# LuoGuiwen/MSM_blst

Measured on AMD Instinct MI355X. Metric: G1 MSM point-scalar pairs/sec at n=2^20, 1/2/4/8 MI355X; bit-exact vs CPU, higher is better.
Workload: dtype u32 (exact Fp381 integer arithmetic, 14x28-bit limbs)

## Files before the change

include/msm_mi355x.h:

```cpp
#ifndef MSM_MI355X_H
#define MSM_MI355X_H

#include <stddef.h>
#include <stdint.h>

#ifdef __cplusplus
extern "C" {
#endif

typedef uint8_t byte;
typedef uint64_t limb_t;
typedef struct { byte b[256 / 8]; } blst_scalar;
typedef struct { limb_t l[384 / 8 / sizeof(limb_t)]; } blst_fp;
typedef struct { blst_fp fp[2]; } blst_fp2;
typedef struct { blst_fp x, y, z; } blst_p1;
typedef struct { blst_fp x, y; } blst_p1_affine;
typedef struct { blst_fp2 x, y, z; } blst_p2;
typedef struct { blst_fp2 x, y; } blst_p2_affine;
typedef struct { blst_fp x, y, zzz, zz; } blst_p1xyzz;
typedef struct { blst_fp2 x, y, zzz, zz; } blst_p2xyzz;
typedef struct { int m; int b; int alpha; } digit_decomposition;

size_t blst_p1s_mult_pippenger_scratch_sizeof(size_t npoints);
void blst_p1s_mult_pippenger(blst_p1 *ret, const blst_p1_affine *const points[], size_t npoints,
// ... 242 lines not shown
                    const uint8_t *sig_codes, const uint8_t *key_codes, const uint8_t *late, const uint8_t *is_one,
                    uint8_t *status);

typedef struct { limb_t l[256 / 8 / sizeof(limb_t)]; } blst_fr;
enum { MSM_NTT_INVERSE = 1, MSM_FR_SRC_SCALAR = 2, MSM_FR_DST_SCALAR = 4 };
int msm_fr_ntt(int device, void *dst, const void *src, size_t log_n, size_t batch, const byte *shift, int flags,
               int src_on_device, int dst_on_device, void *hip_stream);
enum { MSM_FR_ADD, MSM_FR_SUB, MSM_FR_MUL, MSM_FR_SQR, MSM_FR_NEG, MSM_FR_INV, MSM_FR_FROM_SCALAR, MSM_FR_TO_SCALAR };
enum { MSM_FR_B_ONE = 1 };
int msm_fr_op(int device, int op, void *dst, const void *a, const void *b, size_t n, int flags, int src_on_device,
              int dst_on_device, void *hip_stream);
int msm_fr_root_of_unity(size_t log_n, blst_fr *out);
int msm_ntt_plan(size_t log_n, int *npasses, int log_radix[], int capacity);
int msm_fr_probe(int device, double out[2]);

enum { MSM_POLY_BITREV = 8 };
int msm_fr_eval_quotient(int device, void *y, void *q, const void *polys, const void *z, size_t log_n, size_t count,
                         int flags, int src_on_device, int dst_on_device, void *hip_stream);
typedef struct msm_kzg_ctx msm_kzg_ctx;
int msm_kzg_ctx_create(msm_kzg_ctx **ctx, int device, size_t log_n, const void *srs_lagrange_g1, int srs_on_device,
                       const void *tau_g2, int flags, void *hip_stream);
void msm_kzg_ctx_destroy(msm_kzg_ctx *ctx);
int msm_kzg_commit(msm_kzg_ctx *ctx, void *dst_affine, const void *polys, size_t count, int src_on_device,
                   int dst_on_device, void *hip_stream);
int msm_kzg_open(msm_kzg_ctx *ctx, void *proofs_affine, void *y, const void *polys, const void *z, size_t count,
                 int src_on_device, int dst_on_device, void *hip_stream);
int msm_kzg_verify(msm_kzg_ctx *ctx, uint8_t *ok, size_t *nfail, const void *commitments, const void *z,
                   const void *y, const void *proofs, size_t count, const byte *weights, size_t nbits,
                   size_t weight_stride, const size_t *batch_offsets, size_t nbatches, int src_on_device,
                   void *hip_stream);

size_t msm_ches_bucket_set(int q, int a_h, int *out, size_t cap);
int msm_ches_digit_table(int q, int a_h, digit_decomposition *out);

void msm_gen_scalars(byte *out32, size_t n, uint64_t seed);
void msm_p1_fixed_points(blst_p1_affine *out, size_t n);
void msm_p2_fixed_points(blst_p2_affine *out, size_t n);
void msm_p1_fixed_points_range(blst_p1_affine *out, size_t start, size_t n);
void msm_p2_fixed_points_range(blst_p2_affine *out, size_t start, size_t n);
void msm_p1_to_affine(blst_p1_affine *out, const blst_p1 *in);
void msm_p2_to_affine(blst_p2_affine *out, const blst_p2 *in);
void msm_p1_compress(byte out[48], const blst_p1 *in);
void msm_p2_compress(byte out[96], const blst_p2 *in);
void msm_p1_add(blst_p1 *out, const blst_p1 *a, const blst_p1 *b);
void msm_p2_add(blst_p2 *out, const blst_p2 *a, const blst_p2 *b);

int msm_test_field(int group, int op, const limb_t *a, const limb_t *b, limb_t *out, size_t n);
int msm_test_xyzz(int group, const void *points_affine, size_t npoints, const uint32_t *ops, int len, size_t nseq,
                  void *out);
int msm_test_fp12(int op, int k, int alias, int raw, const void *a, const void *b, void *out, size_t n);
int msm_test_fp_ops(int field, int form, int op, const uint32_t *in, const uint32_t *flags, uint32_t *out, size_t n,
                    size_t cap);

#ifdef __cplusplus
}
#endif
#endif
```

msm_blst_amd/_ffi.py:

```python
import ctypes
import os

HERE = os.path.dirname(os.path.abspath(__file__))
LIB_PATH = os.path.join(HERE, "libmsm_mi355x.so")

_lib = None


class MsmError(RuntimeError):
    pass


def lib():
    global _lib
    if _lib is not None:
        return _lib
    if not os.path.exists(LIB_PATH):
        raise MsmError(f"{LIB_PATH} not built: run `python -m msm_blst_amd.build` (hipcc, gfx950)")
    L = ctypes.CDLL(LIB_PATH)
    vp, sz, i32, u64 = ctypes.c_void_p, ctypes.c_size_t, ctypes.c_int, ctypes.c_uint64
    for g in (1, 2):
        f = getattr(L, f"blst_p{g}s_mult_pippenger")
        f.argtypes = [vp, vp, sz, vp, sz, vp]
        f.restype = None
        f = getattr(L, f"blst_p{g}s_tile_pippenger")
        f.argtypes = [vp, vp, sz, vp, sz, vp, sz, sz]
        f.restype = None
        f = getattr(L, f"blst_p{g}s_mult_pippenger_scratch_sizeof")
        f.argtypes = [sz]
        f.restype = sz
        getattr(L, f"msm_p{g}_fixed_points").argtypes = [vp, sz]
        getattr(L, f"msm_p{g}_fixed_points_range").argtypes = [vp, sz, sz]
        for name in (f"msm_p{g}_to_affine", f"msm_p{g}_compress"):
            getattr(L, name).argtypes = [vp, vp]
        getattr(L, f"msm_p{g}_add").argtypes = [vp, vp, vp]
    L.msm_last_error.restype = ctypes.c_char_p
    L.msm_device_count.restype = i32
    L.msm_ctx_create.argtypes = [ctypes.POINTER(vp), i32, i32, i32]
    L.msm_ctx_set_points.argtypes = [vp, vp, sz, i32, vp]
    L.msm_ctx_mult.argtypes = [vp, vp, vp, sz, sz, i32, vp]
    L.msm_ctx_mult_batch.argtypes = [vp, vp, vp, sz, sz, sz, sz, i32, vp]
    L.msm_ctx_set_profiling.argtypes = [vp, i32]
    L.msm_ctx_phase_times.argtypes = [vp, vp]
    L.msm_ctx_destroy.argtypes = [vp]
    L.msm_ctx_destroy.restype = None
    L.msm_gen_scalars.argtypes = [vp, sz, u64]
    L.msm_test_field.argtypes = [i32, i32, vp, vp, vp, sz]
    L.msm_test_xyzz.argtypes = [i32, vp, sz, vp, i32, sz, vp]
    L.msm_test_fp12.argtypes = [i32, i32, i32, i32, vp, vp, vp, sz]
    L.msm_test_fp_ops.argtypes = [i32, i32, i32, vp, vp, vp, sz, sz]
    pp = ctypes.POINTER(vp)
    L.msm_ches_params.argtypes = [i32, i32, vp]
    L.msm_ches_ctx_create.argtypes = [pp, i32, i32, i32, i32]
    L.msm_ches_ctx_create_params.argtypes = [pp, i32, i32, vp]
    L.msm_ches_ctx_create_multi.argtypes = [pp, i32, vp, i32, i32, i32]
    L.msm_ches_ctx_shards.argtypes = [vp]
    L.msm_ches_ctx_build_table.argtypes = [vp, vp, sz, i32, vp]
    L.msm_ches_ctx_set_table.argtypes = [vp, vp, sz, i32, vp]
    L.msm_ches_ctx_get_table.argtypes = [vp, vp, sz, sz]
    L.msm_ches_ctx_mult.argtypes = [vp, vp, vp, sz, i32, vp]
    L.msm_ches_ctx_mult_batch.argtypes = [vp, vp, vp, sz, sz, sz, i32, vp]
    L.msm_ches_ctx_set_profiling.argtypes = [vp, i32]
    L.msm_ches_ctx_phase_times.argtypes = [vp, vp]
    L.msm_ches_ctx_bucket_count.argtypes = [vp]
    L.msm_ches_ctx_bucket_count.restype = sz
    L.msm_register_host_table.argtypes = [i32, vp, sz]
    L.msm_unregister_host_table.argtypes = [vp]
    L.msm_ches_ctx_batch_lanes.argtypes = [vp]
    L.msm_ches_ctx_rccl_exchange.argtypes = [vp]
    L.msm_ches_ctx_time_accumulation.argtypes = [vp, vp, sz, i32, i32, vp]
    L.msm_ches_ctx_destroy.argtypes = [vp]
    L.msm_ches_ctx_destroy.restype = None
    L.msm_ches_bucket_set.argtypes = [i32, i32, vp, sz]
    L.msm_ches_bucket_set.restype = sz
    L.msm_ches_digit_table.argtypes = [i32, i32, vp]
    for g in (1, 2):
        f = getattr(L, f"blst_p{g}s_mult_wbits_precompute_sizeof")
        f.argtypes, f.restype = [sz, sz], sz
        f = getattr(L, f"blst_p{g}s_mult_wbits_scratch_sizeof")
        f.argtypes, f.restype = [sz], sz
        f = getattr(L, f"blst_p{g}s_mult_wbits_precompute")
        f.argtypes, f.restype = [vp, sz, vp, sz], None
        f = getattr(L, f"blst_p{g}s_mult_wbits")
        f.argtypes, f.restype = [vp, vp, sz, sz, vp, sz, vp], None
    if hasattr(L, "msm_release_engine_cache"):
        L.msm_release_engine_cache.argtypes = []
        L.msm_release_engine_cache.restype = None
        L.msm_engine_cache_stats.argtypes = [vp]
        L.msm_engine_cache_stats.restype = None
        L.msm_set_engine_cache_limit.argtypes = [sz]
        L.msm_set_engine_cache_limit.restype = sz
    L.msm_set_abort_on_error.argtypes = [i32]
    L.msm_error_pending.argtypes = []
    L.msm_wbits_ctx_create.argtypes = [pp, i32, i32, i32]
    L.msm_wbits_ctx_precompute.argtypes = [vp, vp, sz, i32, vp]
    L.msm_wbits_ctx_set_table.argtypes = [vp, vp, sz, i32, vp]
    L.msm_wbits_ctx_get_table.argtypes = [vp, vp, sz, sz]
    L.msm_wbits_ctx_mult.argtypes = [vp, vp, vp, sz, sz, i32, vp]
    L.msm_wbits_ctx_table_rows.argtypes = [vp]
    L.msm_wbits_ctx_table_rows.restype = sz
    L.msm_wbits_ctx_destroy.argtypes = [vp]
    L.msm_wbits_ctx_destroy.restype = None
    L.msm_bgmw_ctx_create.argtypes = [pp, i32, i32, i32, i32]
# ... 67 lines not shown
```

msm_blst_amd/csrc/abi.cpp:

```cpp
#include <hip/hip_runtime.h>
#include <stdio.h>
#include <stdlib.h>
#include <string.h>

#include <algorithm>
#include <atomic>
#include <map>
#include <memory>
#include <mutex>
#include <string>
#include <type_traits>
#include <utility>
#include <vector>

#include "../../include/msm_mi355x.h"
#include "decode.hpp"
#include "encode.hpp"
#include "engine.hpp"
#include "fr_ntt.hpp"
#include "fp_ops_test.hpp"
#include "fr_poly.hpp"
#include "hash_to_curve.hpp"
#include "host_fr.hpp"
#include "kzg.hpp"
// ... 1914 lines not shown

int msm_test_field(int group, int op, const limb_t *a, const limb_t *b, limb_t *out, size_t n) {
  return guarded(MSM_E_HIP, [&] {
    by_group(group, [&](auto g) { test_field<decltype(g)::value>(op, a, b, out, n); });
    return MSM_OK;
  });
}
int msm_test_xyzz(int group, const void *pts, size_t npts, const uint32_t *ops, int len, size_t nseq, void *out) {
  return guarded(MSM_E_HIP, [&] {
    by_group(group, [&](auto g) {
      test_xyzz<decltype(g)::value>((const uint64_t *)pts, npts, ops, len, nseq, (uint64_t *)out);
    });
    return MSM_OK;
  });
}
int msm_test_fp12(int op, int k, int alias, int raw, const void *a, const void *b, void *out, size_t n) {
  if (op < TEST_FP12_MUL || op > TEST_FP12_LINE_ADD) return fail(MSM_E_ARG, "unknown op");
  if (op == TEST_FP12_FROB && (k < 1 || k > 3)) return fail(MSM_E_ARG, "Frobenius power outside 1..3");
  if (op == TEST_FP12_CSQR && (k < 1 || k > 64)) return fail(MSM_E_ARG, "squaring count outside 1..64");
  const bool binary = op == TEST_FP12_MUL || op == TEST_FP12_SPARSE;
  const bool alias_ok = alias == 0 || (alias == 1 && op <= TEST_FP12_CSQR && op != TEST_FP12_INV) ||
                        (alias == 2 && op == TEST_FP12_MUL);
  if (!alias_ok || (raw != 0 && raw != 1)) return fail(MSM_E_ARG, "bad alias / raw");
  if (n && (!a || !out || (binary && !b))) return fail(MSM_E_ARG, "null operand");
  if (!n) return MSM_OK;
  if (!device_ok(0)) return no_device();
  return guarded(MSM_E_HIP, [&] {
    test_fp12(op, k, alias, raw != 0, a, binary ? b : nullptr, out, n);
    return MSM_OK;
  });
}
int msm_test_fp_ops(int field, int form, int op, const uint32_t *in, const uint32_t *flags, uint32_t *out, size_t n,
                    size_t cap) {
  const TestFpOp *d = test_fp_op(op);
  if (!d) return fail(MSM_E_ARG, "unknown op");
  if (field < TEST_FIELD_FP || field > TEST_FIELD_FP2L) return fail(MSM_E_ARG, "unknown field");
  if (form != TEST_FORM_SPLIT && form != TEST_FORM_CHAIN) return fail(MSM_E_ARG, "unknown form");
  if (form == TEST_FORM_CHAIN && (!d->forms || field != TEST_FIELD_FP))
    return fail(MSM_E_ARG, "no single-chain form of this op on this field");
  if (d->fp_only && field != TEST_FIELD_FP) return fail(MSM_E_ARG, "an Fp-only op");
  if ((op == TEST_COOP_ADD || op == TEST_F_MUL_SUB_BS) && field == TEST_FIELD_FP2)
    return fail(MSM_E_ARG, "the one-lane Fp2 has no f_mul_sub_bs and no cooperative kernel");
  if (cap < n) return fail(MSM_E_ARG, "cap < n");
  if (n && ((d->nin && !in) || (d->flags && !flags) || !out)) return fail(MSM_E_ARG, "null operand");
  if (!n) return MSM_OK;
  if (!device_ok(0)) return no_device();
  return guarded(MSM_E_HIP, [&] {
    if (op != TEST_COOP_ADD) test_fp_ops(field, form, op, in, flags, out, n, cap);
    else if (field == TEST_FIELD_FP) test_coop_pair_add<1>(in, out, n, cap);
    else test_coop_pair_add<2>(in, out, n, cap);
    return MSM_OK;
  });
}

int msm_wbits_ctx_create(msm_wbits_ctx **ctx, int group, int device, int wbits) {
  if (!ctx || (group != 1 && group != 2)) return fail(MSM_E_ARG, "bad ctx/group");
  if (!device_ok(device)) return no_device();
  return create_ctx(ctx, group, device, MSM_E_ARG,
                    [&](auto g) { return std::make_unique<Wbits<decltype(g)::value>>(device, wbits); });
}

int msm_wbits_ctx_precompute(msm_wbits_ctx *ctx, const void *pts, size_t n, int on_device, void *stream) {
  if (!ctx || (!pts && n)) return fail(MSM_E_ARG, "bad args");
  return set_table_ctx(ctx, [&](auto &e) { e.precompute(pts, n, on_device != 0, (hipStream_t)stream); });
}

int msm_wbits_ctx_set_table(msm_wbits_ctx *ctx, const void *tab, size_t n, int on_device, void *stream) {
  if (!ctx || (!tab && n)) return fail(MSM_E_ARG, "bad args");
  return set_table_ctx(ctx, [&](auto &e) { e.set_table(tab, n, on_device != 0, (hipStream_t)stream); });
}

int msm_wbits_ctx_get_table(msm_wbits_ctx *ctx, void *out, size_t first, size_t count) {
  return get_table_ctx(ctx, out, first, count, MSM_E_ARG);
}

int msm_wbits_ctx_mult(msm_wbits_ctx *ctx, void *ret, const byte *scalars, size_t stride, size_t nbits,
                       int on_device, void *stream) {
  if (!ctx || !ret || stride == 0 || (nbits + 7) / 8 > stride) return fail(MSM_E_ARG, "bad args (stride < nbits/8)");
  if (!ctx->ready) return fail(MSM_E_STATE, "no table: precompute or set_table first");
  return guarded(MSM_E_HIP, [&] {
    DeviceGuard g(ctx->device);
    hipStream_t s = (hipStream_t)stream;
    ctx->with([&](auto &e) {
      const uint8_t *d = stage_scalars(ctx->scalars, scalars, e.npoints() * stride, on_device != 0, s);
      mult_out(e, ret, 1, [&](auto *out) { e.run(s, d, stride, (int)nbits, out); });
    });
    return MSM_OK;
  });
}

size_t msm_wbits_ctx_table_rows(const msm_wbits_ctx *ctx) {
  return ctx ? ctx->with([](auto &e) { return e.table_rows(); }) : 0;
}

void msm_wbits_ctx_destroy(msm_wbits_ctx *ctx) { delete ctx; }

}
```

msm_blst_amd/csrc/batch_plan.hpp:

```cpp
#pragma once
#include <stddef.h>
#include <stdint.h>

#include <algorithm>
#include <cstdlib>
#include <vector>

namespace msm {

inline std::vector<size_t> front_groups(size_t count, size_t fg_max) {
  std::vector<size_t> fgb{0};
  while (fgb.back() < count)
    fgb.push_back(std::min(count, fgb.back() + std::min<size_t>(fg_max, std::max<size_t>(1, fgb.back()))));
  return fgb;
}

struct RedGroups {
  size_t count = 0, R = 1;
  RedGroups() = default;
  RedGroups(size_t count_, size_t group_max) : count(count_) {
    const size_t ng = (count + group_max - 1) / group_max;
    R = ng ? (count + ng - 1) / ng : 1;
  }
  size_t groups() const { return (count + R - 1) / R; }
  size_t first(size_t q) const { return std::min(count, q * R); }
  size_t of(size_t k) const { return k / R; }
  size_t slot(size_t k) const { return k % R; }
  bool ends(size_t k) const { return (k + 1) % R == 0 || k + 1 == count; }
};

struct BatchKnobs {
  bool tail_coop = true;
  int red_group = 0, pip_group = 0;
  bool bit_tail = true;
  int front_group = 0, pip_front_group = 4;
  bool acc_group = true;
  int h2d_slots = 0;
  int copy_pace = 8;
  int acc_after_l0 = -1;
  int batch_lanes = 0;
  int fine_bt = 1024, pip_fine_bt = 1024;
  int batch_l0_chunk = 8, pip_l0_chunk = 0;

  static int env_int(const char *name, int unset, int lo, int hi) {
    const char *e = getenv(name);
    return e ? std::max(lo, std::min(hi, atoi(e))) : unset;
  }
  static int env_flag(const char *name, int unset) {
    const char *e = getenv(name);
    return e ? atoi(e) != 0 : unset;
  }
  static int env_bt(const char *name) {
    const char *e = getenv(name);
    return e && atoi(e) == 256 ? 256 : 1024;
  }
  static const BatchKnobs &env() {
    static const BatchKnobs k = [] {
      BatchKnobs b;
      b.tail_coop = env_flag("MSM_TAIL_COOP", 1);
      b.red_group = env_int("MSM_RED_GROUP", 0, 1, 32);
      b.pip_group = env_int("MSM_PIP_GROUP", 0, 1, 32);
      b.bit_tail = env_flag("MSM_BIT_TAIL", 1);
      b.front_group = env_int("MSM_FRONT_GROUP", 0, 1, 8);
      b.pip_front_group = env_int("MSM_PIP_FRONT_GROUP", 4, 1, 8);
      b.acc_group = env_flag("MSM_ACC_GROUP", 1);
      b.h2d_slots = env_int("MSM_H2D_SLOTS", 0, 2, 256);
      b.copy_pace = env_int("MSM_COPY_PACE", 8, 0, 32);
      b.acc_after_l0 = env_flag("MSM_ACC_AFTER_L0", -1);
      b.batch_lanes = env_int("MSM_BATCH_LANES", 0, 1, 3);
      b.fine_bt = env_bt("MSM_FINE_BT");
      b.pip_fine_bt = env_bt("MSM_PIP_FINE_BT");
      b.batch_l0_chunk = env_int("MSM_BATCH_L0_CHUNK", 8, 0, 64);
      b.pip_l0_chunk = env_int("MSM_PIP_L0_CHUNK", 0, 0, 64);
      return b;
    }();
    return k;
  }
};

struct ChesBatch {
  static constexpr int kGroup = 20;
  static constexpr int kFrontGroup = 8;
  static constexpr int kFrontGroupDefault = 1;
  static constexpr int kFronts = 3, kFrontsMax = 5;
  static constexpr int kBSets = 2;
};
struct PlainBatch {
  static constexpr int kFronts = 5, kGroup = 10, kRedSets = 4;
};

enum BatchStream { kCaller = 0, kLane1 = 1, kLane2 = 2, kFront = 3, kCopy = 4, kBatchStreams = 5 };

enum BatchSchedule { kAccGroups, kLanes, kOneLane };

struct BatchShape {
  size_t nsets = 0, nseg = 1;
  size_t n = 0, stride = 32, set_stride = 0;
  int h = 1;
  size_t buckets = 0;
  int lanes = 1, group = 1;
  bool host = false, dev_out = false, bit_tail_ok = false;
  size_t bucket_bytes = 0, out_bytes = 0, bit_bytes = 0;
};

struct BatchPlan {
  size_t count = 0, nseg = 1;
  BatchSchedule sched = kOneLane;
  int lanes = 1;
  bool host = false;
  bool combine_per_group = false;
  size_t jstride = 0;
  bool packed = true;
  RedGroups rg;
  size_t group_max = 1;
  bool bit_tail = false, tail_coop = true, l0_first = false;
  int fine_bt = 1024;
  size_t fg_max = 1, nfg = 0;
  std::vector<size_t> fgb;
  int nfr = 3, nred = 2, bsets = 2;
  size_t sslot = 0, slot_groups = 0, nsg = 0, pace = 0;
  int front_waits = 1;
  size_t out_need = 0, out_alloc = 0, bits_need = 0, bits_alloc = 0;
  size_t bucket_set_bytes = 0;
  int bucket_sets = 2;
// ... 230 lines not shown
```

msm_blst_amd/csrc/bucket_sort.hpp:

```cpp
#pragma once
#include <hip/hip_runtime.h>
#include <stdint.h>

namespace msm {

constexpr int BS_TILE = 4096;
constexpr int BS_MAX_FB_BITS = 12;
constexpr int BS_MAX_CB = 8192;
constexpr uint32_t BS_NONE = 0xffffffffu;
constexpr int SCHED_PER_THREAD = 16;
constexpr int SCHED_PER_BLOCK = 256 * SCHED_PER_THREAD;
__device__ __forceinline__ uint32_t sched_class(uint32_t c) { return 255u - (c < 255u ? c : 255u); }

static __global__ void __launch_bounds__(256)
    k_bs_hist(const uint32_t *__restrict__ keys, size_t ne, int fb_bits, int ncb, int ntiles,
              uint32_t *__restrict__ ghist, uint32_t *__restrict__ classes) {
  __shared__ uint32_t h[BS_MAX_CB];
  keys += (size_t)blockIdx.y * ne;
  ghist += (size_t)blockIdx.y * ncb * ntiles;
  if (blockIdx.x == 0)
    for (int c = threadIdx.x; c < 512; c += blockDim.x) classes[(size_t)blockIdx.y * 512 + c] = 0;
  for (int b = threadIdx.x; b < ncb; b += blockDim.x) h[b] = 0;
  __syncthreads();
  const size_t t0 = (size_t)blockIdx.x * BS_TILE;
// ... 75 lines not shown
    sv[pos] = vv[r];
  }
  __syncthreads();
  for (uint32_t i = threadIdx.x; i < total; i += 256) {
    const uint32_t k = sk[i], b = k >> fb_bits;
    const uint32_t g = gb[b] + (i - loff[b]);
    okeys[g] = k;
    ovals[g] = sv[i];
  }
}

template <int BT>
__device__ __forceinline__ void block_exclusive_scan_4096(uint32_t *a, int n, uint32_t *wsum) {
  constexpr int PER = 4096 / BT, NW = BT / 64;
  const int t = threadIdx.x, lane = t & 63, wave = t >> 6;
  const int per = (n + BT - 1) / BT;
  uint32_t loc[PER], s = 0;
#pragma unroll
  for (int k = 0; k < PER; ++k) {
    int i = t * per + k;
    loc[k] = s;
    if (k < per && i < n) s += a[i];
  }
  uint32_t incl = s;
#pragma unroll
  for (int d = 1; d < 64; d <<= 1) {
    uint32_t v = __shfl_up(incl, d, 64);
    if (lane >= d) incl += v;
  }
  if (lane == 63) wsum[wave] = incl;
  __syncthreads();
  if (t == 0) {
    uint32_t run = 0;
    for (int w = 0; w < NW; ++w) {
      uint32_t x = wsum[w];
      wsum[w] = run;
      run += x;
    }
  }
  __syncthreads();
  const uint32_t base = wsum[wave] + incl - s;
#pragma unroll
  for (int k = 0; k < PER; ++k) {
    int i = t * per + k;
    if (k < per && i < n) a[i] = base + loc[k];
  }
  __syncthreads();
}

constexpr int BS_FINE_CAP = 30 * 1024;
constexpr int BS_FINE_STEP = BS_FINE_CAP - BS_FINE_CAP / 8;
constexpr int BS_FINE_MAXW = 8;

template <int BT>
static __global__ void __launch_bounds__(BT)
    k_bs_fine(const uint32_t *__restrict__ okeys, const uint32_t *__restrict__ ovals, int fb_bits, int ncb,
              int ntiles, const uint32_t *__restrict__ gbase, const uint32_t *__restrict__ ghist, uint32_t nb,
              uint32_t *__restrict__ sorted, uint32_t *__restrict__ counts, uint32_t *__restrict__ offsets,
              uint32_t *__restrict__ class_total, int nsets) {
  __shared__ uint32_t off[1 << BS_MAX_FB_BITS];
  __shared__ uint8_t win[1 << BS_MAX_FB_BITS];
  __shared__ uint32_t stage[BS_FINE_CAP];
  __shared__ uint32_t wsum[BT / 64];
  __shared__ uint32_t wb[BS_FINE_MAXW + 1];
  __shared__ uint32_t cls[256];
  const int FB = 1 << fb_bits;
  const uint32_t fmask = (uint32_t)FB - 1u;
  const int b = blockIdx.x, set = blockIdx.y;
  const size_t per = (size_t)ncb * ntiles, s0 = (size_t)set * per;
  const size_t last = (size_t)nsets * per - 1;
  const uint32_t lo = gbase[s0 + (size_t)b * ntiles];
  const uint32_t hi = b + 1 < ncb ? gbase[s0 + (size_t)(b + 1) * ntiles]
                                  : (set + 1 < nsets ? gbase[s0 + per] : gbase[last] + ghist[last]);
  counts += (size_t)set * nb;
  offsets += (size_t)set * nb;
  class_total += (size_t)set * 512;
  const uint32_t nbin = hi - lo;
  for (int f = threadIdx.x; f < FB; f += blockDim.x) off[f] = 0;
  for (int c = threadIdx.x; c < 256; c += BT) cls[c] = 0;
  if (threadIdx.x <= BS_FINE_MAXW) wb[threadIdx.x] = nbin;
  __syncthreads();
  constexpr int U = 16, UW = 12;
  for (uint32_t e0 = lo; e0 < hi; e0 += U * BT) {
    uint32_t kk[U];
#pragma unroll
    for (int r = 0; r < U; ++r) {
      uint32_t e = e0 + threadIdx.x + r * BT;
      kk[r] = e < hi ? okeys[e] : BS_NONE;
    }
#pragma unroll
    for (int r = 0; r < U; ++r)
      if (kk[r] != BS_NONE) atomicAdd(&off[kk[r] & fmask], 1u);
  }
  __syncthreads();
  for (int f = threadIdx.x; f < FB; f += blockDim.x) {
    uint32_t bucket = ((uint32_t)b << fb_bits) + f;
    if (bucket < nb) {
      counts[bucket] = off[f];
      atomicAdd(&cls[sched_class(off[f])], 1u);
    }
  }
  __syncthreads();
  for (int c = threadIdx.x; c < 256; c += BT)
    if (cls[c]) atomicAdd(&class_total[c], cls[c]);
  block_exclusive_scan_4096<BT>(off, FB, wsum);
  const uint32_t nwin = (nbin + BS_FINE_STEP - 1) / BS_FINE_STEP;
  const bool staged = nwin <= (uint32_t)BS_FINE_MAXW;
  for (int f = threadIdx.x; f < FB; f += blockDim.x) {
    uint32_t bucket = ((uint32_t)b << fb_bits) + f;
    if (bucket < nb) offsets[bucket] = lo + off[f];
    if (staged) {
      uint32_t w = off[f] / BS_FINE_STEP;
      win[f] = (uint8_t)w;
      atomicMin(&wb[w], off[f]);
    }
  }
  __syncthreads();
  if (!staged) {
    for (uint32_t e0 = lo; e0 < hi; e0 += U * BT) {
      uint32_t kk[U], vv[U];
#pragma unroll
      for (int r = 0; r < U; ++r) {
        uint32_t e = e0 + threadIdx.x + r * BT;
        kk[r] = e < hi ? okeys[e] : BS_NONE;
        vv[r] = e < hi ? ovals[e] : 0u;
      }
#pragma unroll
      for (int r = 0; r < U; ++r) {
        if (kk[r] == BS_NONE) continue;
        uint32_t pos = atomicAdd(&off[kk[r] & fmask], 1u);
        sorted[lo + pos] = vv[r];
      }
    }
    return;
  }
  for (uint32_t k = 0; k < nwin; ++k) {
    const uint32_t base = wb[k];
    if (base == nbin) continue;
    uint32_t end = nbin;
    for (uint32_t j = k + 1; j < nwin; ++j)
      if (wb[j] < end) end = wb[j];
    for (uint32_t e0 = lo; e0 < hi; e0 += UW * BT) {
      uint32_t kk[UW], vv[UW];
#pragma unroll
      for (int r = 0; r < UW; ++r) {
        uint32_t e = e0 + threadIdx.x + r * BT;
        kk[r] = e < hi ? okeys[e] : BS_NONE;
        vv[r] = e < hi ? ovals[e] : 0u;
      }
#pragma unroll
      for (int r = 0; r < UW; ++r) {
        if (kk[r] == BS_NONE || win[kk[r] & fmask] != k) continue;
        uint32_t li = atomicAdd(&off[kk[r] & fmask], 1u) - base;
        if (li < (uint32_t)BS_FINE_CAP)
          stage[li] = vv[r];
        else
          sorted[lo + base + li] = vv[r];
      }
    }
    __syncthreads();
    const uint32_t nst = min(end - base, (uint32_t)BS_FINE_CAP);
    for (uint32_t i = threadIdx.x; i < nst; i += BT) sorted[lo + base + i] = stage[i];
    __syncthreads();
  }
}

static __global__ void __launch_bounds__(256, 6)
    k_sched_scatter(const uint32_t *__restrict__ counts, const uint32_t *__restrict__ offsets, uint32_t nb,
                    uint32_t *__restrict__ class_total, uint32_t *__restrict__ order, uint32_t *__restrict__ scnt,
                    uint32_t *__restrict__ soff) {
  __shared__ uint32_t h[256];
  __shared__ uint32_t base[256];
  __shared__ uint32_t wsum[4];
  counts += (size_t)blockIdx.y * nb;
  offsets += (size_t)blockIdx.y * nb;
  order += (size_t)blockIdx.y * nb;
  scnt += (size_t)blockIdx.y * nb;
  soff += (size_t)blockIdx.y * nb;
  class_total += (size_t)blockIdx.y * 512;
  const uint32_t t = threadIdx.x, b0 = blockIdx.x * SCHED_PER_BLOCK, lane = t & 63, wave = t >> 6;
  h[t] = 0;
  const uint32_t v = class_total[t];
  uint32_t incl = v;
#pragma unroll
  for (int d = 1; d < 64; d <<= 1) {
// ... 92 lines not shown
```

msm_blst_amd/csrc/engine.hip:

```cpp
#include <hipcub/hipcub.hpp>

#include <algorithm>

#include "bucket_sort.hpp"
#include "engine.hpp"
#include "hoststage.hpp"
#include "kernels.hpp"
#include "pair_kernels.hpp"

#ifndef MSM_GROUP
#error "define MSM_GROUP (1 or 2)"
#endif

namespace msm {

#if MSM_GROUP == 1
BucketSort::Geom BucketSort::prepare(hipStream_t s, size_t ne, uint32_t nb, int nsets, int ntiles) {
  Geom g;
  g.fb_bits = 8;
  while (g.fb_bits < BS_MAX_FB_BITS && ((size_t)nb >> g.fb_bits) > 384) ++g.fb_bits;
  g.ncb = (int)(((size_t)nb + (1u << g.fb_bits) - 1) >> g.fb_bits);
  if (g.ncb > BS_MAX_CB || g.ncb > 4096) throw std::runtime_error("BucketSort: too many buckets");
  if (nsets < 1 || nsets > 65535) throw std::runtime_error("BucketSort: bad set count");
  if (ne * nsets >= (1ull << 32)) throw std::runtime_error("BucketSort: too many entries");
  g.ntiles = ntiles > 0 ? ntiles : (int)std::max<size_t>(1, (ne + BS_TILE - 1) / BS_TILE);
  g.nslots = (size_t)nsets * g.ncb * g.ntiles;
  if (g.nslots >= (1ull << 31)) throw std::runtime_error("BucketSort: too many histogram slots");
  ghist.ensure(g.nslots * 4);
  gbase.ensure(g.nslots * 4);
  okeys.ensure(std::max<size_t>(ne * nsets, 1) * 4);
  ovals.ensure(std::max<size_t>(ne * nsets, 1) * 4);
  wbase.ensure(groups(nb) * nsets * 4);
  ipay_stride = ne + BS_IPAY_SLACK;
  ipay.ensure(ipay_stride * nsets * 4);
  size_t scan_tmp = 0;
  hipcub::DeviceScan::ExclusiveSum(nullptr, scan_tmp, ghist.as<uint32_t>(), gbase.as<uint32_t>(), (int)g.nslots, s);
  tmp.ensure(scan_tmp);
  g.scan_tmp = scan_tmp;
  classes.ensure((size_t)512 * 4 * nsets);
  scnt.ensure((size_t)nb * nsets * 4);
  soff.ensure((size_t)nb * nsets * 4);
  return g;
}

void BucketSort::scan(hipStream_t s, const Geom &g) {
  size_t tb = g.scan_tmp;
  MSM_HIP_CHECK(
      hipcub::DeviceScan::ExclusiveSum(tmp.p, tb, ghist.as<uint32_t>(), gbase.as<uint32_t>(), (int)g.nslots, s));
}

void BucketSort::run(hipStream_t s, const uint32_t *keys, const uint32_t *vals, size_t ne, uint32_t nb,
                     uint32_t *sorted, uint32_t *counts, uint32_t *offsets, uint32_t *order, int nsets) {
  const Geom g = prepare(s, ne, nb, nsets, 0);
  hipLaunchKernelGGL(k_bs_hist, dim3(g.ntiles, nsets), dim3(256), 0, s, keys, ne, g.fb_bits, g.ncb, g.ntiles,
                     ghist.as<uint32_t>(), classes.as<uint32_t>());
  MSM_HIP_CHECK(hipGetLastError());
  scan(s, g);
  hipLaunchKernelGGL(k_bs_coarse, dim3(g.ntiles, nsets), dim3(256), (size_t)(2 * g.ncb + 2 * BS_TILE) * 4, s, keys,
                     vals, ne, g.fb_bits, g.ncb, g.ntiles, gbase.as<uint32_t>(), okeys.as<uint32_t>(),
                     ovals.as<uint32_t>());
  MSM_HIP_CHECK(hipGetLastError());
  finish(s, g, ne, nb, sorted, counts, offsets, order, nsets);
}

void BucketSort::finish(hipStream_t s, const Geom &g, size_t ne, uint32_t nb, uint32_t *sorted, uint32_t *counts,
                        uint32_t *offsets, uint32_t *order, int nsets) {
  (void)ne;
  const int fb_bits = g.fb_bits, ncb = g.ncb, ntiles = g.ntiles;
  const size_t nw = groups(nb);
  if (fine_bt == 256)
    hipLaunchKernelGGL(k_bs_fine<256>, dim3(ncb, nsets), dim3(256), 0, s, okeys.as<uint32_t>(),
                       ovals.as<uint32_t>(), fb_bits, ncb, ntiles, gbase.as<uint32_t>(), ghist.as<uint32_t>(), nb,
                       sorted, counts, offsets, classes.as<uint32_t>(), nsets);
  else
    hipLaunchKernelGGL(k_bs_fine<1024>, dim3(ncb, nsets), dim3(1024), 0, s, okeys.as<uint32_t>(),
                       ovals.as<uint32_t>(), fb_bits, ncb, ntiles, gbase.as<uint32_t>(), ghist.as<uint32_t>(), nb,
                       sorted, counts, offsets, classes.as<uint32_t>(), nsets);
  MSM_HIP_CHECK(hipGetLastError());
  hipLaunchKernelGGL(k_sched_scatter, dim3(nblk(nb, SCHED_PER_BLOCK), nsets), dim3(256), 0, s, counts, offsets, nb,
                     classes.as<uint32_t>(), order, scnt.as<uint32_t>(), soff.as<uint32_t>());
  MSM_HIP_CHECK(hipGetLastError());
  hipLaunchKernelGGL(k_interleave, dim3((unsigned)nw / 4 + 1, nsets), dim3(256), 0, s, scnt.as<uint32_t>(),
                     soff.as<uint32_t>(), nb, (uint32_t)nw, classes.as<uint32_t>(), sorted, ipay.as<uint32_t>(),
                     ipay_stride, wbase.as<uint32_t>());
  MSM_HIP_CHECK(hipGetLastError());
}
#endif


template <int G>
Pippenger<G>::Pippenger(int device, int window_bits) : dev_(device), c_(window_bits) {
  if (c_ < 8 || c_ > 20) throw std::runtime_error("window_bits out of range [8,20]");
  DeviceGuard g(dev_);
  ev_.resize(8);
  for (auto &e : ev_) MSM_HIP_CHECK(hipEventCreate(&e));
}
template <int G>
Pippenger<G>::~Pippenger() {
  for (auto &e : ev_) (void)hipEventDestroy(e);
  for (auto &e : bev_) (void)hipEventDestroy(e);
  for (hipStream_t q : {fstream_, lane1_, tstream_})
    if (q) {
      (void)hipStreamSynchronize(q);
      (void)hipStreamDestroy(q);
    }
  if (host_out_) (void)hipHostFree(host_out_);
  if (up_) {
    (void)hipStreamSynchronize(up_);
    (void)hipStreamDestroy(up_);
    (void)hipEventDestroy(ev_up_);
    (void)hipEventDestroy(ev_s_);
  }
}

template <int G>
size_t Pippenger<G>::device_bytes() const {
  size_t b = stage_ ? stage_->pinned_bytes() : 0;
  for (const DevBuf *d : {&pts_, &buckets_[0], &buckets_[1], &gbuckets_[0], &gbuckets_[1], &tmp_, &scal_}) b += d->bytes;
  for (const ChesFrontSet &f : fs_) b += f.device_bytes();
  return b + red_.device_bytes() + (batch_red_ != &red_ ? bred_.device_bytes() : 0);
}

template <int G>
void Pippenger<G>::set_points(const void *pts, size_t n, bool on_device, hipStream_t s) {
  typedef typename FieldOf<G>::F F;
  DeviceGuard g(dev_);
  if (n == 0) {
    n_ = 0;
    return;
  }
  if (n >= (1ull << 31)) throw std::runtime_error("too many points");
  size_t raw = n * 96 * G;
  const void *src = pts;
  if (!on_device) {
    tmp_.ensure(raw);
    MSM_HIP_CHECK(hipMemcpyAsync(tmp_.p, pts, raw, hipMemcpyHostToDevice, s));
    src = tmp_.p;
  }
// ... 433 lines not shown
```

msm_blst_amd/csrc/engine.hpp:

```cpp
#pragma once
#include <hip/hip_runtime.h>
#include <stdint.h>

#include <cstdlib>
#include <memory>
#include <stdexcept>
#include <string>
#include <vector>

#include "acc_sched.hpp"
#include "batch_plan.hpp"
#include "ches_setup.hpp"
#include "host_fp.hpp"
#include "reduce_plan.hpp"

#define MSM_HIP_CHECK(x)                                                                           \
  do {                                                                                            \
    hipError_t e_ = (x);                                                                          \
    if (e_ != hipSuccess)                                                                         \
      throw std::runtime_error(std::string("HIP error ") + hipGetErrorString(e_) + " at " + #x); \
  } while (0)

namespace msm {

class HostStager;

inline unsigned nblk(size_t n, unsigned b) { return (unsigned)((n + b - 1) / b); }

struct DevBuf {
  void *p = nullptr;
  size_t bytes = 0;
  DevBuf() = default;
  DevBuf(const DevBuf &) = delete;
  DevBuf &operator=(const DevBuf &) = delete;
  DevBuf(DevBuf &&o) noexcept : p(o.p), bytes(o.bytes) { o.p = nullptr, o.bytes = 0; }
  ~DevBuf() { release(); }
  void release() {
    if (p) (void)hipFree(p);
    p = nullptr;
    bytes = 0;
  }
  void ensure(size_t b) {
    if (b <= bytes) return;
    release();
    MSM_HIP_CHECK(hipMalloc(&p, b));
    bytes = b;
  }
  template <class T>
  T *as() const {
    return reinterpret_cast<T *>(p);
  }
};

struct PhaseTimes {
  float digits = 0, sort = 0, accumulate = 0, reduce = 0, finalize = 0, total = 0;
  int accumulate_launches = 0;
};

template <int G>
struct HostField;
template <>
struct HostField<1> {
  typedef hfp::Fp F;
};
template <>
struct HostField<2> {
  typedef hfp::Fp2 F;
};

struct BucketSort {
  DevBuf ghist, gbase, okeys, ovals, classes, tmp;
  DevBuf scnt, soff, wbase, ipay;
  size_t ipay_stride = 0;
  int fine_bt = 1024;
  static size_t groups(size_t nb) { return (nb + 63) / 64; }
  AccSched sched(const uint32_t *order, const uint32_t *sorted, size_t set, size_t nb) const {
    const size_t nw = groups(nb);
    return AccSched{order + set * nb,
                    scnt.as<uint32_t>() + set * nb,
                    soff.as<uint32_t>() + set * nb,
                    wbase.as<uint32_t>() + set * nw,
                    ipay.as<uint32_t>() + set * ipay_stride,
                    sorted};
  }
  AccStride stride(size_t nb) const { return AccStride{nb, groups(nb), ipay_stride}; }
  void run(hipStream_t s, const uint32_t *keys, const uint32_t *vals, size_t ne, uint32_t nb, uint32_t *sorted,
           uint32_t *counts, uint32_t *offsets, uint32_t *order, int nsets = 1);
  struct Geom {
    int fb_bits = 8, ncb = 1, ntiles = 1;
    size_t nslots = 0, scan_tmp = 0;
  };
  Geom prepare(hipStream_t s, size_t ne, uint32_t nb, int nsets, int ntiles);
  void scan(hipStream_t s, const Geom &g);
  void finish(hipStream_t s, const Geom &g, size_t ne, uint32_t nb, uint32_t *sorted, uint32_t *counts,
              uint32_t *offsets, uint32_t *order, int nsets);
  size_t device_bytes() const {
    return ghist.bytes + gbase.bytes + okeys.bytes + ovals.bytes + classes.bytes + tmp.bytes + scnt.bytes + soff.bytes +
           wbase.bytes + ipay.bytes;
  }
};

template <class HF>
hfp::Jac<HF> horner(const std::vector<hfp::Jac<HF>> &T, int c) {
  hfp::Jac<HF> ret = T.back();
  for (int w = (int)T.size() - 2; w >= 0; --w) {
    for (int k = 0; k < c; ++k) ret = hfp::dbl(ret);
    ret = hfp::addj(ret, T[w]);
  }
  return ret;
}



template <int G>
struct ScanReducer {
  typedef typename HostField<G>::F HF;
  DevBuf buf[2], fin;
  void launch(hipStream_t s, const void *A, int W, int S, bool coop = true);
};

template <int G>
class WeightedReducer {
 public:
  typedef typename HostField<G>::F HF;
  static constexpr int NSETS = 4;
  void plan(const std::vector<uint32_t> &w, const std::vector<uint32_t> &win, int nwin, int c0 = 0);
  void plan(const std::vector<uint32_t> &w, int c0 = 0) { plan(w, {}, 1, c0); }
  int level0_chunk() const { return plan_.c0; }
  void ensure(int set, int nmsm);
  void head(hipStream_t s, const void *S, size_t sstride, int set, int slot0, int nmsm);
  void tail(hipStream_t s, int set, int nmsm, ReduceEnding end, bool coop);
  void copy_out(hipStream_t s, int set, int nmsm, ReduceEnding end, void *dst, hipMemcpyKind kind = hipMemcpyDefault);
  size_t out_bytes() const { return (size_t)2 * plan_.nwin * 144 * G; }
  size_t bit_bytes() const { return plan_.bit_slots() * 144 * G; }
  bool has_bit_tail() const { return plan_.has_bit_tail(); }
  std::vector<hfp::Jac<HF>> combine(const void *host) const;
  hfp::Jac<HF> combine_bits(const void *host) const;
  hfp::Jac<HF> combine_windows(const void *host, int c) const;
  void launch(hipStream_t s, const void *S) {
    ensure(0, 1);
    head(s, S, size(), 0, 0, 1);
    tail(s, 0, 1, sync_ending(), true);
  }
  std::vector<hfp::Jac<HF>> read_windows(hipStream_t s);
  hfp::Jac<HF> read(hipStream_t s) { return read_windows(s)[0]; }
  hfp::Jac<HF> read_total(hipStream_t s, int c);
  size_t size() const { return plan_.nbuckets; }
  size_t device_bytes() const {
    size_t b = idx_.bytes;
    for (const DevBuf &d : starts_) b += d.bytes;
    for (int t = 0; t < NSETS; ++t)
      b += dense_buf_[t].bytes + part_[t][0].bytes + part_[t][1].bytes + bgfin_[t].bytes + dense_[t].buf[0].bytes +
           dense_[t].buf[1].bytes + dense_[t].fin.bytes;
// ... 243 lines not shown
```

Measured before the change: 459.2 million.

## Keep bin keys in registers in fine bucket sort to read once

Adds a template variant of the fine bucket-sort kernel that loads each bin's keys into registers once, captures the atomic rank during the counting pass, and reuses the packed rank and window in the scatter pass instead of re-reading keys and doing a second atomic. It is enabled by default for the 1024-thread path when a bin fits in 56 keys per thread. The intent is to cut global key traffic and LDS atomics in the sort stage. The cost is much higher register pressure, which may lower occupancy, and a fallback path for oversized bins. A test entry point is also added.

```diff
diff --git a/include/msm_mi355x.h b/include/msm_mi355x.h
--- a/include/msm_mi355x.h
+++ b/include/msm_mi355x.h
@@ -318,6 +318,9 @@
 int msm_test_fp_ops(int field, int form, int op, const uint32_t *in, const uint32_t *flags, uint32_t *out, size_t n,
                     size_t cap);
 
+int msm_test_bucket_sort(const uint32_t *keys, const uint32_t *vals, size_t ne, uint32_t nb, int nsets, int variant,
+                         uint32_t *counts, uint32_t *offsets, uint32_t *sorted, uint32_t *geom);
+
 #ifdef __cplusplus
 }
 #endif
diff --git a/msm_blst_amd/_ffi.py b/msm_blst_amd/_ffi.py
--- a/msm_blst_amd/_ffi.py
+++ b/msm_blst_amd/_ffi.py
@@ -49,6 +49,7 @@
     L.msm_test_xyzz.argtypes = [i32, vp, sz, vp, i32, sz, vp]
     L.msm_test_fp12.argtypes = [i32, i32, i32, i32, vp, vp, vp, sz]
     L.msm_test_fp_ops.argtypes = [i32, i32, i32, vp, vp, vp, sz, sz]
+    L.msm_test_bucket_sort.argtypes = [vp, vp, sz, ctypes.c_uint32, i32, i32, vp, vp, vp, vp]
     pp = ctypes.POINTER(vp)
     L.msm_ches_params.argtypes = [i32, i32, vp]
     L.msm_ches_ctx_create.argtypes = [pp, i32, i32, i32, i32]
diff --git a/msm_blst_amd/csrc/abi.cpp b/msm_blst_amd/csrc/abi.cpp
--- a/msm_blst_amd/csrc/abi.cpp
+++ b/msm_blst_amd/csrc/abi.cpp
@@ -1990,6 +1990,18 @@
     return MSM_OK;
   });
 }
+int msm_test_bucket_sort(const uint32_t *keys, const uint32_t *vals, size_t ne, uint32_t nb, int nsets, int variant,
+                         uint32_t *counts, uint32_t *offsets, uint32_t *sorted, uint32_t *geom) {
+  if (variant != 0 && variant != 1) return fail(MSM_E_ARG, "unknown variant");
+  if (nb < 1 || nsets < 1 || nsets > 65535) return fail(MSM_E_ARG, "bad bucket / set count");
+  if (ne && ne * (size_t)nsets >= (1ull << 32) / 4) return fail(MSM_E_ARG, "too many entries");
+  if (!counts || !offsets || (ne && (!keys || !vals || !sorted))) return fail(MSM_E_ARG, "null operand");
+  if (!device_ok(0)) return no_device();
+  return guarded(MSM_E_HIP, [&] {
+    test_bucket_sort(keys, vals, ne, nb, nsets, variant, counts, offsets, sorted, geom);
+    return MSM_OK;
+  });
+}
 
 int msm_wbits_ctx_create(msm_wbits_ctx **ctx, int group, int device, int wbits) {
   if (!ctx || (group != 1 && group != 2)) return fail(MSM_E_ARG, "bad ctx/group");
diff --git a/msm_blst_amd/csrc/batch_plan.hpp b/msm_blst_amd/csrc/batch_plan.hpp
--- a/msm_blst_amd/csrc/batch_plan.hpp
+++ b/msm_blst_amd/csrc/batch_plan.hpp
@@ -40,6 +40,7 @@
   int acc_after_l0 = -1;
   int batch_lanes = 0;
   int fine_bt = 1024, pip_fine_bt = 1024;
+  bool fine_one_read = true;
   int batch_l0_chunk = 8, pip_l0_chunk = 0;
 
   static int env_int(const char *name, int unset, int lo, int hi) {
@@ -70,6 +71,7 @@
       b.batch_lanes = env_int("MSM_BATCH_LANES", 0, 1, 3);
       b.fine_bt = env_bt("MSM_FINE_BT");
       b.pip_fine_bt = env_bt("MSM_PIP_FINE_BT");
+      b.fine_one_read = env_flag("MSM_FINE_ONE_READ", 1);
       b.batch_l0_chunk = env_int("MSM_BATCH_L0_CHUNK", 8, 0, 64);
       b.pip_l0_chunk = env_int("MSM_PIP_L0_CHUNK", 0, 0, 64);
       return b;
diff --git a/msm_blst_amd/csrc/bucket_sort.hpp b/msm_blst_amd/csrc/bucket_sort.hpp
--- a/msm_blst_amd/csrc/bucket_sort.hpp
+++ b/msm_blst_amd/csrc/bucket_sort.hpp
@@ -151,7 +151,9 @@
 constexpr int BS_FINE_STEP = BS_FINE_CAP - BS_FINE_CAP / 8;
 constexpr int BS_FINE_MAXW = 8;
 
-template <int BT>
+constexpr int BS_FINE_KEYS = 56;
+constexpr int BS_FINE_VALS = 28;
+template <int BT, int E = 0>
 static __global__ void __launch_bounds__(BT)
     k_bs_fine(const uint32_t *__restrict__ okeys, const uint32_t *__restrict__ ovals, int fb_bits, int ncb,
               int ntiles, const uint32_t *__restrict__ gbase, const uint32_t *__restrict__ ghist, uint32_t nb,
@@ -180,16 +182,42 @@
   if (threadIdx.x <= BS_FINE_MAXW) wb[threadIdx.x] = nbin;
   __syncthreads();
   constexpr int U = 16, UW = 12;
-  for (uint32_t e0 = lo; e0 < hi; e0 += U * BT) {
-    uint32_t kk[U];
-#pragma unroll
-    for (int r = 0; r < U; ++r) {
-      uint32_t e = e0 + threadIdx.x + r * BT;
-      kk[r] = e < hi ? okeys[e] : BS_NONE;
-    }
-#pragma unroll
-    for (int r = 0; r < U; ++r)
-      if (kk[r] != BS_NONE) atomicAdd(&off[kk[r] & fmask], 1u);
+  constexpr int EK = E > 0 ? E : 1;
+  static_assert((size_t)E * BT <= 0x10000, "rank and position are packed in 16 bits");
+  static_assert(((size_t)E * BT + BS_FINE_STEP - 1) / BS_FINE_STEP <= (size_t)BS_FINE_MAXW, "always staged");
+  const bool regs = E > 0 && nbin <= (uint32_t)(E * BT);
+  uint32_t ek[EK];
+  if (regs) {
+    const uint32_t *bk = okeys + lo;
+#pragma unroll
+    for (int r = 0; r < EK; ++r) {
+      const uint32_t i = threadIdx.x + r * BT;
+      ek[r] = i < nbin ? bk[i] : BS_NONE;
+    }
+    constexpr int A = 14;
+#pragma unroll
+    for (int c = 0; c < EK; c += A) {
+      uint32_t rk[A];
+#pragma unroll
+      for (int j = 0; j < A; ++j)
+        if (c + j < EK)
+          rk[j] = atomicAdd(ek[c + j] != BS_NONE ? &off[ek[c + j] & fmask] : &stage[threadIdx.x], 1u);
+#pragma unroll
+      for (int j = 0; j < A; ++j)
+        if (c + j < EK && ek[c + j] != BS_NONE) ek[c + j] = (ek[c + j] & fmask) | rk[j] << BS_MAX_FB_BITS;
+    }
+  } else {
+    for (uint32_t e0 = lo; e0 < hi; e0 += U * BT) {
+      uint32_t kk[U];
+#pragma unroll
+      for (int r = 0; r < U; ++r) {
+        uint32_t e = e0 + threadIdx.x + r * BT;
+        kk[r] = e < hi ? okeys[e] : BS_NONE;
+      }
+#pragma unroll
+      for (int r = 0; r < U; ++r)
+        if (kk[r] != BS_NONE) atomicAdd(&off[kk[r] & fmask], 1u);
+    }
   }
   __syncthreads();
   for (int f = threadIdx.x; f < FB; f += blockDim.x) {
@@ -230,6 +258,49 @@
         uint32_t pos = atomicAdd(&off[kk[r] & fmask], 1u);
         sorted[lo + pos] = vv[r];
       }
+    }
+    return;
+  }
+  if (regs) {
+#pragma unroll
+    for (int r = 0; r < EK; ++r) {
+      const uint32_t o = off[ek[r] & (uint32_t)((1 << BS_MAX_FB_BITS) - 1)];
+      const uint32_t pw = (o + (ek[r] >> BS_MAX_FB_BITS)) | (o / BS_FINE_STEP) << 16;
+      ek[r] = ek[r] != BS_NONE ? pw : BS_NONE;
+    }
+    const uint32_t *bv = ovals + lo;
+    constexpr int V = BS_FINE_VALS < EK ? BS_FINE_VALS : EK;
+    for (uint32_t k = 0; k < nwin; ++k) {
+      const uint32_t base = wb[k];
+      if (base == nbin) continue;
+      uint32_t end = nbin;
+      for (uint32_t j = k + 1; j < nwin; ++j)
+        if (wb[j] < end) end = wb[j];
+      uint32_t t = threadIdx.x;
+      asm volatile("" : "+v"(t));
+      t &= BT - 1;
+#pragma unroll
+      for (int r = 0; r < EK; ++r) asm volatile("" : "+v"(ek[r]));
+#pragma unroll
+      for (int c = 0; c < EK; c += V) {
+        uint32_t vv[V];
+#pragma unroll
+        for (int j = 0; j < V; ++j)
+          if (c + j < EK) vv[j] = (ek[c + j] >> 16) == k ? bv[t + (c + j) * BT] : 0u;
+#pragma unroll
+        for (int j = 0; j < V; ++j) {
+          if (c + j >= EK || (ek[c + j] >> 16) != k) continue;
+          const uint32_t li = (ek[c + j] & 0xffffu) - base;
+          if (li < (uint32_t)BS_FINE_CAP)
+            stage[li] = vv[j];
+          else
+            sorted[lo + base + li] = vv[j];
+        }
+      }
+      __syncthreads();
+      const uint32_t nst = min(end - base, (uint32_t)BS_FINE_CAP);
+      for (uint32_t i = threadIdx.x; i < nst; i += BT) sorted[lo + base + i] = stage[i];
+      __syncthreads();
     }
     return;
   }
diff --git a/msm_blst_amd/csrc/engine.hip b/msm_blst_amd/csrc/engine.hip
--- a/msm_blst_amd/csrc/engine.hip
+++ b/msm_blst_amd/csrc/engine.hip
@@ -72,6 +72,10 @@
     hipLaunchKernelGGL(k_bs_fine<256>, dim3(ncb, nsets), dim3(256), 0, s, okeys.as<uint32_t>(),
                        ovals.as<uint32_t>(), fb_bits, ncb, ntiles, gbase.as<uint32_t>(), ghist.as<uint32_t>(), nb,
                        sorted, counts, offsets, classes.as<uint32_t>(), nsets);
+  else if (fine_one_read)
+    hipLaunchKernelGGL((k_bs_fine<1024, BS_FINE_KEYS>), dim3(ncb, nsets), dim3(1024), 0, s, okeys.as<uint32_t>(),
+                       ovals.as<uint32_t>(), fb_bits, ncb, ntiles, gbase.as<uint32_t>(), ghist.as<uint32_t>(), nb,
+                       sorted, counts, offsets, classes.as<uint32_t>(), nsets);
   else
     hipLaunchKernelGGL(k_bs_fine<1024>, dim3(ncb, nsets), dim3(1024), 0, s, okeys.as<uint32_t>(),
                        ovals.as<uint32_t>(), fb_bits, ncb, ntiles, gbase.as<uint32_t>(), ghist.as<uint32_t>(), nb,
@@ -84,6 +88,32 @@
                      soff.as<uint32_t>(), nb, (uint32_t)nw, classes.as<uint32_t>(), sorted, ipay.as<uint32_t>(),
                      ipay_stride, wbase.as<uint32_t>());
   MSM_HIP_CHECK(hipGetLastError());
+}
+
+void test_bucket_sort(const uint32_t *keys, const uint32_t *vals, size_t ne, uint32_t nb, int nsets, int variant,
+                      uint32_t *counts, uint32_t *offsets, uint32_t *sorted, uint32_t *geom) {
+  DeviceGuard g(0);
+  BucketSort bs;
+  bs.fine_bt = 1024, bs.fine_one_read = variant == 1;
+  const size_t nen = ne * nsets, nbn = (size_t)nb * nsets;
+  DevBuf dk, dv, ds, dc, dof, dor;
+  dk.ensure(std::max<size_t>(nen, 1) * 4), dv.ensure(std::max<size_t>(nen, 1) * 4);
+  ds.ensure(nen * 4 + 64), dc.ensure(nbn * 4), dof.ensure(nbn * 4), dor.ensure(nbn * 4);
+  if (nen) {
+    MSM_HIP_CHECK(hipMemcpy(dk.p, keys, nen * 4, hipMemcpyHostToDevice));
+    MSM_HIP_CHECK(hipMemcpy(dv.p, vals, nen * 4, hipMemcpyHostToDevice));
+  }
+  MSM_HIP_CHECK(hipMemset(ds.p, 0xff, nen * 4 + 64));
+  bs.run(nullptr, dk.as<uint32_t>(), dv.as<uint32_t>(), ne, nb, ds.as<uint32_t>(), dc.as<uint32_t>(),
+         dof.as<uint32_t>(), dor.as<uint32_t>(), nsets);
+  MSM_HIP_CHECK(hipStreamSynchronize(nullptr));
+  MSM_HIP_CHECK(hipMemcpy(counts, dc.p, nbn * 4, hipMemcpyDeviceToHost));
+  MSM_HIP_CHECK(hipMemcpy(offsets, dof.p, nbn * 4, hipMemcpyDeviceToHost));
+  if (nen) MSM_HIP_CHECK(hipMemcpy(sorted, ds.p, nen * 4, hipMemcpyDeviceToHost));
+  if (geom) {
+    const BucketSort::Geom gm = bs.prepare(nullptr, ne, nb, nsets, 0);
+    geom[0] = (uint32_t)gm.fb_bits, geom[1] = BS_FINE_KEYS * 1024, geom[2] = BS_FINE_CAP, geom[3] = BS_FINE_STEP;
+  }
 }
 #endif
 
diff --git a/msm_blst_amd/csrc/engine.hpp b/msm_blst_amd/csrc/engine.hpp
--- a/msm_blst_amd/csrc/engine.hpp
+++ b/msm_blst_amd/csrc/engine.hpp
@@ -73,6 +73,7 @@
   DevBuf scnt, soff, wbase, ipay;
   size_t ipay_stride = 0;
   int fine_bt = 1024;
+  bool fine_one_read = BatchKnobs::env().fine_one_read;
   static size_t groups(size_t nb) { return (nb + 63) / 64; }
   AccSched sched(const uint32_t *order, const uint32_t *sorted, size_t set, size_t nb) const {
     const size_t nw = groups(nb);
@@ -99,6 +100,9 @@
            wbase.bytes + ipay.bytes;
   }
 };
+
+void test_bucket_sort(const uint32_t *keys, const uint32_t *vals, size_t ne, uint32_t nb, int nsets, int variant,
+                      uint32_t *counts, uint32_t *offsets, uint32_t *sorted, uint32_t *geom);
 
 template <class HF>
 hfp::Jac<HF> horner(const std::vector<hfp::Jac<HF>> &T, int c) {
```

Result: no change. 460.1 million (median of 5 runs) (+0.2%).
